# rohitgandikota/sliders

Hardware: AMD Instinct MI355X
Metric: UNet denoise steps/sec (SDXL rank-4 text slider) (higher is better)
Workload: dtype bf16; 1 GPU; sdxl text slider rank=4 alpha=1 noxattn+c3lier, 1024x1024, batch 1 (CFG pair), DDIM-50 partial denoise k~U{1..49} + 4 predictions + backward + AdamW; bench_step=one training iteration, prompt_pairs=8, parallelism=dp1

## Files before the change

sliders_amd/csrc/common.h:

```cpp
#pragma once
#include <hip/hip_runtime.h>
#include <stdint.h>

typedef __attribute__((ext_vector_type(8))) __bf16 bf16x8;
typedef __attribute__((ext_vector_type(4))) __bf16 bf16x4;
typedef __attribute__((ext_vector_type(2))) __bf16 bf16x2;
typedef __attribute__((ext_vector_type(16))) float f32x16;
typedef __attribute__((ext_vector_type(2))) float f32x2;
typedef __attribute__((ext_vector_type(4))) float f32x4;
typedef __attribute__((ext_vector_type(4))) unsigned int u32x4;
typedef __attribute__((ext_vector_type(2))) unsigned int u32x2;

typedef unsigned short bf16_t;

#define SLH_WAVE 64

static __device__ __attribute__((aligned(64))) unsigned int slh_zero_page[64];

__device__ __forceinline__ float bf2f(__bf16 x) { return (float)x; }
__device__ __forceinline__ __bf16 f2bf(float x) { return (__bf16)x; }

__device__ __forceinline__ float bfraw2f(unsigned short u) {
    return __builtin_bit_cast(float, ((unsigned int)u) << 16);
}
__device__ __forceinline__ unsigned short f2bfraw(float f) {
    return __builtin_bit_cast(unsigned short, (__bf16)f);
}
__device__ __forceinline__ float round_bf16(float f) { return (float)((__bf16)f); }

__device__ __forceinline__ float silu_f(float x) { return x / (1.0f + __expf(-x)); }
__device__ __forceinline__ float gelu_erf_f(float x) { return 0.5f * x * (1.0f + erff(x * 0.70710678118654752f)); }
__device__ __forceinline__ float gelu_erf_fast_f(float x) {
    const float z = fabsf(x) * 0.70710678118654752f;
    const float t = __builtin_amdgcn_rcpf(__builtin_fmaf(0.5f, z, 1.0f));
    float p = 0.17087277f;
    p = __builtin_fmaf(p, t, -0.82215223f); p = __builtin_fmaf(p, t, 1.48851587f); p = __builtin_fmaf(p, t, -1.13520398f);
    p = __builtin_fmaf(p, t, 0.27886807f); p = __builtin_fmaf(p, t, -0.18628806f); p = __builtin_fmaf(p, t, 0.09678418f);
    p = __builtin_fmaf(p, t, 0.37409196f); p = __builtin_fmaf(p, t, 1.00002368f); p = __builtin_fmaf(p, t, -1.26551223f);
    const float e = t * __expf(__builtin_fmaf(-z, z, p));
    const float h = 0.5f * e;
    return x * (x >= 0.f ? 1.0f - h : h);
}

__device__ __forceinline__ float wave_sum(float v) {
#pragma unroll
    for (int o = 32; o > 0; o >>= 1) v += __shfl_xor(v, o, 64);
    return v;
}
__device__ __forceinline__ float wave_max(float v) {
#pragma unroll
    for (int o = 32; o > 0; o >>= 1) v = fmaxf(v, __shfl_xor(v, o, 64));
    return v;
}

__device__ __forceinline__ void glds16(const void* gsrc, void* lds_wave_base) {
    __builtin_amdgcn_global_load_lds((const __attribute__((address_space(1))) void*)gsrc,
                                     (__attribute__((address_space(3))) void*)lds_wave_base, 16, 0, 0);
}

__device__ __forceinline__ void lds_dma_syncthreads() {
    asm volatile("s_waitcnt vmcnt(0)" ::: "memory");
    __syncthreads();
}

__device__ __forceinline__ void glds16_hidden(const void* gsrc, unsigned lds_byte_addr) {
    asm volatile("s_mov_b32 m0, %1\n\ts_nop 0\n\tglobal_load_lds_dwordx4 %0, off" ::"v"(gsrc), "s"(lds_byte_addr) : "memory");
}
__device__ __forceinline__ unsigned lds_addr_of(const void* p) {
    return (unsigned)(uintptr_t)(const __attribute__((address_space(3))) char*)p;
}
__device__ __forceinline__ int lds_off(int row, int slot) {
    return row * 128 + ((slot ^ ((row >> 1) & 7)) << 4);
}

__device__ __forceinline__ int batch_find(const int* prefix, int n, int bid) {
    int lo = 0, hi = n;
    while (hi - lo > 1) {
        const int mid = (lo + hi) >> 1;
        if (prefix[mid] <= bid) lo = mid; else hi = mid;
    }
    return lo;
// ... 142 lines not shown
#pragma unroll
            for (int u = 0; u < U; ++u) { a += (double)v[u][0]; b += (double)v[u][1]; }
        }
    }
    for (int o = lpg >> 1; o > 0; o >>= 1) {
        a += __shfl_xor(a, o, 64);
        b += __shfl_xor(b, o, 64);
    }
    S = a; Q = b;
}

__device__ __forceinline__ bool gn_cluster_reduce(const GnWorkspace ws, float* rows, unsigned* tickets, int rb, int groups, int lpg, int g,
                                                  bool owner, float S1, float Q1, int* lds_flag, double& S, double& Q) {
    const int cl = ws.cluster_of(rb);
    if (owner) store_pair_sc1(ws.pair(rows, groups, rb, g), S1, Q1);
    const int members = ws.members(cl);
    if (!last_arriver(ws.cluster_ticket(tickets, cl), (unsigned)members, lds_flag)) return false;
    gn_combine_partials(ws.pair(rows, groups, ws.first(cl), 0), members, groups, lpg, S, Q);
    return true;
}
__device__ __forceinline__ bool gn_two_level_reduce(const GnWorkspace ws, float* rows, unsigned* tickets, int rb, int groups, int lpg,
                                                    bool owner, float S1, float Q1, int* lds_flag, double& S, double& Q) {
    const int tid = threadIdx.x;
    const int g = tid / lpg;
    if (!gn_cluster_reduce(ws, rows, tickets, rb, groups, lpg, g, owner, S1, Q1, lds_flag, S, Q)) return false;
    if (ws.clusters() == 1) return g < groups && (tid & (lpg - 1)) == 0;
    if (g < groups && (tid & (lpg - 1)) == 0) store_pair_sc1(ws.pair(rows, groups, ws.cluster_row(ws.cluster_of(rb)), g), (float)S, (float)Q);
    if (!last_arriver(ws.level2_ticket(tickets), (unsigned)ws.clusters(), lds_flag)) return false;
    gn_combine_partials(ws.pair(rows, groups, ws.cluster_row(0), 0), ws.clusters(), groups, lpg, S, Q);
    return g < groups && (tid & (lpg - 1)) == 0;
}

__device__ __forceinline__ f32x2 gn_finish(double S, double Q, int hw, int cg, double pivot, float eps) {
    const double n = (double)hw * (double)cg;
    const double m = S / n;
    const double var = fmax(Q / n - m * m, 0.0);
    return f32x2{(float)(pivot + m), (float)(1.0 / sqrt(var + (double)eps))};
}

void slh_set_error(const char* fmt, ...);
#define SLH_CHECK(cond, ...)            \
    do {                                \
        if (!(cond)) {                  \
            slh_set_error(__VA_ARGS__); \
            return -1;                  \
        }                               \
    } while (0)
bool slh_name_mode();
void slh_name_record(const char* fmt, ...);
void slh_name_sink_set(char* buf, int cap);
void slh_launch_record(int grid, int block, const void* args, size_t bytes);
void slh_launch_recorded(int* grid, int* block, unsigned long long* args_hash);
inline const char* slh_tf(bool b) { return b ? "true" : "false"; }
template <auto Kern, class A, class... N>
inline void slh_launch(int grid, int block, hipStream_t s, const A& a, const char* fmt, N... n) {
    if (slh_name_mode()) { slh_name_record(fmt, n...); slh_launch_record(grid, block, &a, sizeof(A)); return; }
    hipLaunchKernelGGL(Kern, dim3(grid), dim3(block), 0, s, a);
}
#define SLH_LAUNCH_CHECK(name)                                              \
    do {                                                                    \
        if (slh_name_mode()) break;                                         \
        hipError_t e_ = hipGetLastError();                                  \
        if (e_ != hipSuccess) {                                             \
            slh_set_error("%s: launch failed: %s", name, hipGetErrorString(e_)); \
            return -2;                                                      \
        }                                                                   \
    } while (0)
```

sliders_amd/csrc/lora.hip:

```cpp
#include "addressing.h"
#include "../../include/sliders_hip.h"

namespace {

struct AddrArgs {
    const __bf16* a0; const __bf16* a1;
    int lda0, lda1, ca0, ca1;
    int mode, hs, ws, src_xform, stride, ho, wo;
};

template <int RMAX, int LPR>
__global__ __launch_bounds__(256) void skinny_kernel(AddrArgs A, const __bf16* __restrict__ w,
                                                     const __bf16* __restrict__ bias, void* out,
                                                     int M, int R, int K, int ldo, int out_kind, int kmajor) {
    const int tid = threadIdx.x;
    const int sub = tid & (LPR - 1);
    const int m = blockIdx.x * (256 / LPR) + tid / LPR;
    const bool active = m < M;
    const int mm = active ? m : M - 1;
    float acc[RMAX];
#pragma unroll
    for (int r = 0; r < RMAX; ++r) acc[r] = 0.f;
    const int cin = A.ca0 + A.ca1;

// ... 37 lines not shown
            const bf16x8 nxt = *(const bf16x8*)src_of(k + LPR * 8);
            fma_chunk(cur, k);
            cur = nxt;
        }
    } else {
        const int hw = A.ho * A.wo;
        const int b = mm / hw;
        const int rem = mm - b * hw;
        const int oy = rem / A.wo, ox = rem - oy * A.wo;
        const int sh = A.src_xform ? 1 : 0;
        const int HL = A.hs << sh, WL = A.ws << sh;
        for (int tap = 0; tap < 9; ++tap) {
            const int ky = tap / 3, kx = tap - ky * 3;
            const int iy = oy * A.stride + ky - 1, ix = ox * A.stride + kx - 1;
            bool ok = (iy >= 0) & (iy < HL) & (ix >= 0) & (ix < WL);
            if (A.src_xform == 2) ok = ok & (((iy | ix) & 1) == 0);
            if (!ok) continue;
            const long pix = ((long)b * A.hs + (iy >> sh)) * A.ws + (ix >> sh);
            auto src_of = [&](int c) {
                const int cc = c < cin ? c : 0;
                return cc < A.ca0 ? A.a0 + pix * A.lda0 + cc : A.a1 + pix * A.lda1 + (cc - A.ca0);
            };
            bf16x8 cur = *(const bf16x8*)src_of(sub * 8);
            for (int c = sub * 8; c < cin; c += LPR * 8) {
                const bf16x8 nxt = *(const bf16x8*)src_of(c + LPR * 8);
                fma_chunk(cur, tap * cin + c);
                cur = nxt;
            }
        }
    }
#pragma unroll
    for (int r = 0; r < RMAX; ++r) {
#pragma unroll
        for (int o = LPR / 2; o > 0; o >>= 1) acc[r] += __shfl_xor(acc[r], o, 64);
    }
    if (active && sub == 0) {
        if (out_kind == 0) {
            float* o = (float*)out + (long)m * ldo;
#pragma unroll
            for (int r = 0; r < RMAX; ++r)
                if (r < R) o[r] = acc[r] + (bias ? (float)bias[r] : 0.f);
        } else {
            const int hw = A.ho * A.wo;
            const int b = m / hw;
            const int rem = m - b * hw;
            __bf16* o = (__bf16*)out;
#pragma unroll
            for (int r = 0; r < RMAX; ++r)
                if (r < R) o[((long)b * R + r) * hw + rem] = (__bf16)(acc[r] + (bias ? (float)bias[r] : 0.f));
        }
    }
}

__global__ __launch_bounds__(256) void gemv_kernel(const slh_gemv_desc d) {
    const int lane = threadIdx.x & 63;
    const int n = blockIdx.x * 4 + (threadIdx.x >> 6);
    if (n >= d.N) return;
    const __bf16* x = (const __bf16*)d.x;
    const __bf16* w = (const __bf16*)d.w + (long)n * d.K;
    float acc[8];
#pragma unroll
    for (int b = 0; b < 8; ++b) acc[b] = 0.f;
    for (int k = lane * 8; k < d.K; k += 512) {
        const bf16x8 wv = *(const bf16x8*)(w + k);
        bf16x8 xv[8];
#pragma unroll
        for (int b = 0; b < 8; ++b) xv[b] = *(const bf16x8*)(x + (long)(b < d.nb ? b : d.nb - 1) * d.ldx + k);
        float wf[8];
#pragma unroll
        for (int e = 0; e < 8; ++e) wf[e] = (float)wv[e];
#pragma unroll
        for (int b = 0; b < 8; ++b) {
            if (b < d.nb) {
#pragma unroll
                for (int e = 0; e < 8; ++e) {
                    float xe = (float)xv[b][e];
                    if (d.in_act == 1) xe = round_bf16(silu_f(xe));
                    acc[b] += xe * wf[e];
                }
            }
        }
    }
#pragma unroll
    for (int b = 0; b < 8; ++b) acc[b] = wave_sum(acc[b]);
    if (lane == 0) {
        const float bias = d.bias ? (float)((const __bf16*)d.bias)[n] : 0.f;
        float up[4] = {0.f, 0.f, 0.f, 0.f};
        float ls = 0.f;
        int tcol = 0;
        if (d.lora_t) {
            ls = *d.lora_scale;
            tcol = d.lora_tcol ? d.lora_tcol[n] : 0;
            const bf16x4 u = *(const bf16x4*)((const __bf16*)d.lora_up + (long)n * 4);
#pragma unroll
            for (int r = 0; r < 4; ++r) up[r] = (float)u[r];
        }
        for (int b = 0; b < d.nb; ++b) {
            float v = acc[b] + bias;
            if (d.lora_t) {
                const float* t = d.lora_t + (long)b * d.ld_t + tcol;
                v += ls * (t[0] * up[0] + t[1] * up[1] + t[2] * up[2] + t[3] * up[3]);
            }
            if (d.addend) v = round_bf16(v) + (float)((const __bf16*)d.addend)[(long)b * d.ld_add + n];
            if (d.out_f32) ((float*)d.y)[(long)b * d.ldy + n] = v;
            else ((__bf16*)d.y)[(long)b * d.ldy + n] = (__bf16)v;
        }
    }
}

struct WgradArgs {
    AddrArgs A;
    const float* v; float* out; const float* scale;
    int M, R, ldv, ldo, rows_per_block, rmajor, vgroup_cols;
    float* ws; unsigned* ticket;
};

template <int R>
__device__ __forceinline__ void wgrad_body(const WgradArgs& p, const int bx, const int by, const int bz, const long slab_id = 0,
                                           const int slab_step = 0, const long ticket_id = 0, const int splits = 1) {
    __shared__ float red[4][32][8 * R + 1];
    __shared__ int last_flag;
    const int cx = threadIdx.x & 31, ry = threadIdx.x >> 5;
    const int C = p.A.ca0 + p.A.ca1;
    const int c = (bx * 32 + cx) * 8;
    const bool cvalid = c < C;
    const int tap = bz;
    const int m_begin = by * p.rows_per_block;
    const int m_end = min(p.M, m_begin + p.rows_per_block);
    float acc[8][R];
#pragma unroll
    for (int e = 0; e < 8; ++e)
#pragma unroll
        for (int r = 0; r < R; ++r) acc[e][r] = 0.f;
    const int voff = p.vgroup_cols > 0 ? 4 * (c / p.vgroup_cols) : 0;
    const int ky = tap / 3, kx = tap - ky * 3;
    const SrcSel zs = src_select(p.A, c);
    if (cvalid) {
        for (int m = m_begin + ry; m < m_end; m += 8) {
            long pix = m;
            if (p.A.mode != 0) {
                const RowPixel px = pixel_of_row(m, p.A.ho, p.A.wo);
                const ConvTap t = conv_tap(p.A, px.b, px.oy, px.ox, ky, kx);
                if (!t.ok) continue;
                pix = t.pix;
            }
            const bf16x8 z = *(const bf16x8*)(zs.base + pix * zs.ld + zs.cc);
            float vv[R];
#pragma unroll
            for (int r = 0; r < R; ++r) vv[r] = p.v[(long)m * p.ldv + voff + r];
#pragma unroll
            for (int e = 0; e < 8; ++e) {
                const float ze = (float)z[e];
#pragma unroll
                for (int r = 0; r < R; ++r) acc[e][r] += ze * vv[r];
// ... 108 lines not shown
    p.vgroup_cols = d.vgroup_cols;
    p.ws = d.slabs; p.ticket = (unsigned*)d.tickets;
    p.rows_per_block = wgrad_geom(d.c0 + d.c1, d.M, d.mode, d.slabs ? 1 : 0).rows_per_block;
}

template <int R>
__global__ __launch_bounds__(256) void wgrad_batch_kernel(const slh_wgrad_desc* table, const int* prefix, int n, float* ws, unsigned* ticket) {
    const int bid = blockIdx.x;
    const int pi = __builtin_amdgcn_readfirstlane(batch_find(prefix, n, bid));
    const slh_wgrad_desc d = table[pi];
    WgradArgs p;
    wgrad_args(p, d);
    p.ws = ws; p.ticket = ticket;
    const WgradGeom g = wgrad_geom(d.c0 + d.c1, d.M, d.mode, ws ? 2 : 0);
    p.rows_per_block = g.rows_per_block;
    const int local = bid - prefix[pi];
    const int bx = local % g.gx, rest = local / g.gx;
    const int by = rest % g.splits, bz = rest / g.splits;
    wgrad_body<R>(p, bx, by, bz, bid, g.gx, (long)prefix[pi] + (long)bz * g.splits * g.gx + bx, g.splits);
}

}

struct skinny_form { int rmax, lpr, grid; };
static skinny_form skinny_choose(int M, int R) {
    skinny_form f;
    f.rmax = R <= 4 ? 4 : R <= 12 ? 12 : 16;
    f.lpr = M <= 16384 ? 64 : 16;
    const int rows = 256 / f.lpr;
    f.grid = (M + rows - 1) / rows;
    return f;
}

extern "C" int slh_skinny(const slh_skinny_desc* d, slh_stream_t stream) {
    SLH_CHECK(d && d->a0 && d->w && d->out, "slh_skinny: null pointer");
    SLH_CHECK(d->M > 0 && d->R > 0 && d->R <= 16 && d->K > 0, "slh_skinny: bad shape");
    SLH_CHECK(d->ca0 % 8 == 0 && d->ca1 % 8 == 0 && d->lda0 % 8 == 0 && d->lda1 % 8 == 0 && d->K % 8 == 0,
              "slh_skinny: 16-byte alignment");
    SLH_CHECK((d->a1 != nullptr) == (d->ca1 > 0), "slh_skinny: a1/ca1 mismatch");
    const int cin = d->ca0 + d->ca1;
    if (d->mode == 0) SLH_CHECK(cin == d->K, "slh_skinny: dense K mismatch");
    else {
        SLH_CHECK(d->mode == 1 && d->K == 9 * cin, "slh_skinny: conv K mismatch");
        SLH_CHECK(d->M == d->batch * d->ho * d->wo, "slh_skinny: conv M mismatch");
        SLH_CHECK(d->stride == 1 || d->stride == 2, "slh_skinny: stride");
    }
    if (d->out_kind == 1) SLH_CHECK(d->mode == 1, "slh_skinny: NCHW output needs conv geometry");
    if (d->w_kmajor) SLH_CHECK(d->R == 4 && d->mode == 0 && !d->bias, "slh_skinny: w_kmajor needs dense R=4");
    AddrArgs A;
    fill_addr(A, d->a0, d->a1, d->lda0, d->lda1, d->ca0, d->ca1, d->mode, d->hs, d->ws, d->src_xform, d->stride,
              d->ho, d->wo);
    hipStream_t s = (hipStream_t)stream;
    const skinny_form f = skinny_choose(d->M, d->R);
#define SLH_SKINNY_LAUNCH(RM, LPR)                                                                                 \
    do {                                                                                                           \
        if (slh_name_mode()) slh_name_record("skinny<%d,%d>", RM, LPR);                                            \
        else                                                                                                       \
            hipLaunchKernelGGL((skinny_kernel<RM, LPR>), dim3(f.grid), dim3(256), 0, s, A, (const __bf16*)d->w,    \
                               (const __bf16*)d->bias, d->out, d->M, d->R, d->K, d->ldo, d->out_kind, d->w_kmajor); \
    } while (0)
#define SLH_SKINNY_ROWS(RM)                                                                                        \
    do {                                                                                                           \
        if (f.lpr == 64) SLH_SKINNY_LAUNCH(RM, 64);                                                                \
        else SLH_SKINNY_LAUNCH(RM, 16);                                                                            \
    } while (0)
    if (f.rmax == 4) SLH_SKINNY_ROWS(4);
    else if (f.rmax == 12) SLH_SKINNY_ROWS(12);
    else SLH_SKINNY_ROWS(16);
#undef SLH_SKINNY_ROWS
#undef SLH_SKINNY_LAUNCH
    SLH_LAUNCH_CHECK("slh_skinny");
    return 0;
}

extern "C" int slh_skinny_kernel_name(const slh_skinny_desc* d, char* buf, int cap) {
    SLH_CHECK(buf && cap >= 32, "slh_skinny_kernel_name: buffer");
    slh_name_sink_set(buf, cap);
    const int rc = slh_skinny(d, nullptr);
    slh_name_sink_set(nullptr, 0);
    if (rc == 0 && !buf[0]) { slh_set_error("slh_skinny_kernel_name: internal: no launch site recorded a name"); return -3; }
    return rc;
}

extern "C" int slh_gemv(const slh_gemv_desc* d, slh_stream_t stream) {
    SLH_CHECK(d && d->x && d->w && d->y, "slh_gemv: null pointer");
    SLH_CHECK(d->nb >= 1 && d->nb <= 8 && d->N > 0 && d->K > 0 && d->K % 8 == 0 && d->ldx % 8 == 0,
              "slh_gemv: bad shape nb=%d N=%d K=%d", d->nb, d->N, d->K);
    if (d->lora_t) SLH_CHECK(d->lora_up && d->lora_scale, "slh_gemv: lora pointers");
    hipLaunchKernelGGL(gemv_kernel, dim3((d->N + 3) / 4), dim3(256), 0, (hipStream_t)stream, *d);
    SLH_LAUNCH_CHECK("slh_gemv");
    return 0;
}

static int wgrad_check(const slh_wgrad_desc* d, bool ptrs = true) {
    SLH_CHECK(d, "slh_lora_wgrad: null descriptor");
    if (ptrs) SLH_CHECK(d->z0 && d->v && d->out && d->scale, "slh_lora_wgrad: null pointer");
    SLH_CHECK(d->R == 4 || d->R == 12, "slh_lora_wgrad: R must be 4 or 12");
    SLH_CHECK(d->c0 % 8 == 0 && d->c1 % 8 == 0 && d->ldz0 % 8 == 0 && d->ldz1 % 8 == 0, "slh_lora_wgrad: alignment");
    if (ptrs) SLH_CHECK((d->z1 != nullptr) == (d->c1 > 0), "slh_lora_wgrad: z1/c1 mismatch");
    SLH_CHECK(d->M > 0 && d->c0 + d->c1 > 0, "slh_lora_wgrad: empty problem");
    if (d->mode == 1) SLH_CHECK(d->M == d->batch * d->ho * d->wo, "slh_lora_wgrad: conv M mismatch");
    if (d->vgroup_cols > 0)
        SLH_CHECK(d->vgroup_cols % 8 == 0 && (d->c0 + d->c1) % d->vgroup_cols == 0 && d->R == 4,
                  "slh_lora_wgrad: vgroup_cols %d needs a multiple of 8 that divides C = %d, and R = 4 (R = %d)", d->vgroup_cols,
                  d->c0 + d->c1, d->R);
    SLH_CHECK(d->vgroup_cols >= 0, "slh_lora_wgrad: negative vgroup_cols");
    return 0;
}

extern "C" int slh_lora_wgrad(const slh_wgrad_desc* d, slh_stream_t stream) {
    if (wgrad_check(d)) return -1;
    WgradArgs p;
    wgrad_args(p, *d);
    SLH_CHECK((d->slabs != nullptr) == (d->tickets != nullptr), "slh_lora_wgrad: slabs and tickets come together");
    const WgradGeom g = wgrad_geom(d->c0 + d->c1, d->M, d->mode, d->slabs ? 1 : 0);
    dim3 grid(g.gx, g.splits, g.taps);
    hipStream_t s = (hipStream_t)stream;
    if (d->R == 4) hipLaunchKernelGGL(wgrad_kernel<4>, grid, dim3(256), 0, s, p);
    else hipLaunchKernelGGL(wgrad_kernel<12>, grid, dim3(256), 0, s, p);
    SLH_LAUNCH_CHECK("slh_lora_wgrad");
    return 0;
}

extern "C" int slh_lora_wgrad_blocks(const slh_wgrad_desc* d) {
    if (wgrad_check(d, false)) return -1;
    const WgradGeom g = wgrad_geom(d->c0 + d->c1, d->M, d->mode, d->slabs ? 2 : 0);
    return g.gx * g.splits * g.taps;
}

extern "C" int slh_lora_wgrad_single_blocks(const slh_wgrad_desc* d) {
    if (wgrad_check(d, false)) return -1;
    const WgradGeom g = wgrad_geom(d->c0 + d->c1, d->M, d->mode, 1);
    return g.gx * g.splits * g.taps;
}

extern "C" int slh_lora_wgrad_geometry(const slh_wgrad_desc* d, int kind, int32_t* out4) {
    if (wgrad_check(d, false)) return -1;
    SLH_CHECK(kind >= 0 && kind <= 2 && out4, "slh_lora_wgrad_geometry: kind must be 0, 1 or 2");
    const WgradGeom g = wgrad_geom(d->c0 + d->c1, d->M, d->mode, kind);
    out4[0] = g.gx; out4[1] = g.splits; out4[2] = g.taps; out4[3] = g.rows_per_block;
    return 0;
}
// ... 147 lines not shown
```

sliders_amd/csrc/ops.hip:

```cpp
#include "common.h"
#include "../../include/sliders_hip.h"

namespace {

__global__ void tembed_kernel(const slh_tembed_desc d) {
    const int idx = blockIdx.x * blockDim.x + threadIdx.x;
    const int per = d.n_vals * d.dim;
    if (idx >= d.nb * per) return;
    const int b = idx / per;
    const int rem = idx - b * per;
    const int j = rem / d.dim;
    const int i = rem - j * d.dim;
    const int half = d.dim / 2;
    const int fi = i < half ? i : i - half;
    const float exponent = (-9.210340371976184f * (float)fi) / (float)half;
    const float arg = d.vals[b * d.n_vals + j] * expf(exponent);
    const float v = i < half ? cosf(arg) : sinf(arg);
    ((__bf16*)d.out)[(long)b * d.ldo + d.col0 + rem] = (__bf16)v;
}

constexpr int CONVIN_ITERS = 8;
__global__ void conv_in_kernel(const slh_convin_desc d, int nchunk, int ppb) {
    extern __shared__ __attribute__((aligned(16))) char cin_smem[];
    __bf16* sw = (__bf16*)cin_smem;
// ... 8 lines not shown
    const long npix = (long)d.batch * hw;
    float bias[8];
#pragma unroll
    for (int e = 0; e < 8; ++e) bias[e] = d.bias ? (float)((const __bf16*)d.bias)[chunk * 8 + e] : 0.f;
    for (int it = 0; it < CONVIN_ITERS; ++it) {
        const long pix = ((long)blockIdx.x * CONVIN_ITERS + it) * ppb + pl;
        if (pix >= npix) break;
        const int b = (int)(pix / hw);
        const int rem = (int)(pix - (long)b * hw);
        const int oy = rem / d.wd, ox = rem - oy * d.wd;
        const __bf16* x = (const __bf16*)d.x + (long)b * d.cin * hw;
        float acc[8];
#pragma unroll
        for (int e = 0; e < 8; ++e) acc[e] = bias[e];
        if (d.cin <= 4) {
            __bf16 xin[9][4];
            bool tin[9];
#pragma unroll
            for (int tap = 0; tap < 9; ++tap) {
                const int iy = oy + tap / 3 - 1, ix = ox + tap % 3 - 1;
                tin[tap] = iy >= 0 && iy < d.h && ix >= 0 && ix < d.wd;
                const int cy = iy < 0 ? 0 : (iy >= d.h ? d.h - 1 : iy), cx = ix < 0 ? 0 : (ix >= d.wd ? d.wd - 1 : ix);
#pragma unroll
                for (int ci = 0; ci < 4; ++ci) xin[tap][ci] = x[(long)(ci < d.cin ? ci : 0) * hw + cy * d.wd + cx];
            }
#pragma unroll
            for (int tap = 0; tap < 9; ++tap) {
                if (!tin[tap]) continue;
#pragma unroll
                for (int ci = 0; ci < 4; ++ci) {
                    if (ci >= d.cin) break;
                    const float xv = (float)xin[tap][ci];
                    const bf16x8 wv = *(const bf16x8*)(sw + (tap * d.cin + ci) * d.cout + chunk * 8);
#pragma unroll
                    for (int e = 0; e < 8; ++e) acc[e] += xv * (float)wv[e];
                }
            }
        } else {
            for (int tap = 0; tap < 9; ++tap) {
                const int iy = oy + tap / 3 - 1, ix = ox + tap % 3 - 1;
                if (iy < 0 || iy >= d.h || ix < 0 || ix >= d.wd) continue;
                for (int ci = 0; ci < d.cin; ++ci) {
                    const float xv = (float)x[(long)ci * hw + iy * d.wd + ix];
                    const bf16x8 wv = *(const bf16x8*)(sw + (tap * d.cin + ci) * d.cout + chunk * 8);
#pragma unroll
                    for (int e = 0; e < 8; ++e) acc[e] += xv * (float)wv[e];
                }
            }
        }
        bf16x8 o;
#pragma unroll
        for (int e = 0; e < 8; ++e) o[e] = (__bf16)acc[e];
        *(bf16x8*)((__bf16*)d.y + pix * d.ldy + chunk * 8) = o;
    }
}

__global__ __launch_bounds__(256) void ew_kernel(const slh_ew_desc d) {
    const int nchunk = d.C / 8;
    const long gid = (long)blockIdx.x * blockDim.x + threadIdx.x;
    if (gid >= (long)d.M * nchunk) return;
    const int chunk = (int)(gid % nchunk);
    const long m = gid / nchunk;
    const int c = chunk * 8;
    const __bf16* A = (const __bf16*)d.a;
    const __bf16* B = (const __bf16*)d.b;
    __bf16* O = (__bf16*)d.out;
    if (d.op == SLH_EW_COPY) {
        *(bf16x8*)(O + m * d.ldo + c) = *(const bf16x8*)(A + m * d.lda + c);
    } else if (d.op == SLH_EW_ADD) {
        const bf16x8 x = *(const bf16x8*)(A + m * d.lda + c);
        const bf16x8 y = *(const bf16x8*)(B + m * d.ldb + c);
        bf16x8 o;
#pragma unroll
        for (int e = 0; e < 8; ++e) o[e] = (__bf16)((float)x[e] + (float)y[e]);
        *(bf16x8*)(O + m * d.ldo + c) = o;
    } else if (d.op == SLH_EW_GEGLU_FWD || d.op == SLH_EW_GEGLU_BWD) {
        const int jb = c >> 5, j = c & 31;
        const __bf16* pa = A + m * d.lda + jb * 64 + j;
        const bf16x8 hv = *(const bf16x8*)pa;
        const bf16x8 gv = *(const bf16x8*)(pa + 32);
        if (d.op == SLH_EW_GEGLU_FWD) {
            bf16x8 o;
#pragma unroll
            for (int e = 0; e < 8; ++e) o[e] = (__bf16)((float)hv[e] * round_bf16(gelu_erf_fast_f((float)gv[e])));
            *(bf16x8*)(O + m * d.ldo + c) = o;
        } else {
            const bf16x8 dy = *(const bf16x8*)(B + m * d.ldb + c);
            bf16x8 dh, dg;
#pragma unroll
            for (int e = 0; e < 8; ++e) {
                const float g = (float)gv[e], hh = (float)hv[e], dd = (float)dy[e];
                const float cdf = 0.5f * (1.f + erff(g * 0.70710678118654752f));
                const float pdf = 0.3989422804014327f * __expf(-0.5f * g * g);
                dh[e] = (__bf16)(dd * round_bf16(g * cdf));
                dg[e] = (__bf16)(round_bf16(dd * hh) * (cdf + g * pdf));
            }
            __bf16* po = O + m * d.ldo + jb * 64 + j;
            *(bf16x8*)po = dh;
            *(bf16x8*)(po + 32) = dg;
        }
    } else if (d.op == SLH_EW_UPSAMPLE_BWD) {
        const int w = d.iarg, hw = d.iarg2;
        const long b = m / hw;
        const int rem = (int)(m - b * hw);
        const int y = rem / w, x = rem - y * w;
        const long base = (b * 4 * hw + (long)(2 * y) * (2 * w) + 2 * x);
// ... 131 lines not shown
__global__ __launch_bounds__(256) void adamw_f32_kernel(const slh_adamw_desc d, float decay, float bc2_sqrt,
                                                        float neg_step_size, float w1, float beta2, float w2, float eps) {
    const long i = (long)blockIdx.x * blockDim.x + threadIdx.x;
    if (i >= d.n) return;
    float* P = (float*)d.param; float* M1 = (float*)d.exp_avg; float* M2 = (float*)d.exp_avg_sq;
    const float g = d.grad_scale == 1.0f ? d.grad[i] : d.grad[i] * d.grad_scale;
    float p = P[i] * decay;
    float m = M1[i];
    m = __builtin_fmaf(w1, g - m, m);
    float v = M2[i] * beta2;
    v = __builtin_fmaf(w2, g * g, v);
    float den = __builtin_sqrtf(v);
    den = den / bc2_sqrt;
    den = den + eps;
    p = __builtin_fmaf(neg_step_size, m / den, p);
    P[i] = p; M1[i] = m; M2[i] = v;
    ((__bf16*)d.param_lo)[i] = (__bf16)p;
}

__global__ __launch_bounds__(256) void lion_kernel(const slh_lion_desc d, float decay, float b1, float w1, float b2,
                                                   float w2, float neg_lr) {
    const long i = (long)blockIdx.x * blockDim.x + threadIdx.x;
    if (i >= d.n) return;
    __bf16* P = (__bf16*)d.param; __bf16* M = (__bf16*)d.exp_avg;
    const float g = round_bf16(d.grad[i] * d.grad_scale);
    float p = round_bf16((float)P[i] * decay);
    const float m0 = (float)M[i];
    float u = round_bf16(m0 * b1);
    u = round_bf16(u + w1 * g);
    const float sg = u > 0.f ? 1.f : (u < 0.f ? -1.f : 0.f);
    p = round_bf16(p + neg_lr * sg);
    float m = round_bf16(m0 * b2);
    m = round_bf16(m + w2 * g);
    P[i] = (__bf16)p; M[i] = (__bf16)m;
}

}

extern "C" int slh_timestep_embed(const slh_tembed_desc* d, slh_stream_t stream) {
    SLH_CHECK(d && d->vals && d->out && d->dim % 2 == 0 && d->nb > 0 && d->n_vals > 0, "slh_timestep_embed: bad desc");
    const int total = d->nb * d->n_vals * d->dim;
    hipLaunchKernelGGL(tembed_kernel, dim3((total + 255) / 256), dim3(256), 0, (hipStream_t)stream, *d);
    SLH_LAUNCH_CHECK("slh_timestep_embed");
    return 0;
}

extern "C" int slh_conv_in(const slh_convin_desc* d, slh_stream_t stream) {
    SLH_CHECK(d && d->x && d->w && d->y, "slh_conv_in: null pointer");
    SLH_CHECK(d->cout % 8 == 0 && d->ldy % 8 == 0 && d->cin > 0 && d->cin <= 16, "slh_conv_in: bad shape");
    const int nchunk = d->cout / 8;
    SLH_CHECK(nchunk <= 256 && 9 * d->cin * d->cout * 2 <= 64 * 1024, "slh_conv_in: weights must fit 64 KB of LDS");
    const int ppb = 256 / nchunk;
    const long npix = (long)d->batch * d->h * d->wd;
    const long per_block = (long)ppb * CONVIN_ITERS;
    hipLaunchKernelGGL(conv_in_kernel, dim3((unsigned)((npix + per_block - 1) / per_block)), dim3(nchunk * ppb),
                       9 * d->cin * d->cout * 2, (hipStream_t)stream, *d, nchunk, ppb);
    SLH_LAUNCH_CHECK("slh_conv_in");
    return 0;
}

extern "C" int slh_elementwise(const slh_ew_desc* d, slh_stream_t stream) {
    SLH_CHECK(d && d->a && d->out, "slh_elementwise: null pointer");
    SLH_CHECK(d->C % 8 == 0 && d->lda % 8 == 0 && d->ldo % 4 == 0, "slh_elementwise: alignment");
    hipStream_t s = (hipStream_t)stream;
    if (d->op == SLH_EW_COLSUM) {
        SLH_CHECK(d->iarg2 > 0 && d->M % d->iarg2 == 0, "slh_elementwise: colsum rows per sample");
        dim3 grid((d->C / 8 + 31) / 32, (d->iarg2 + 511) / 512, d->M / d->iarg2);
        hipLaunchKernelGGL(colsum_kernel, grid, dim3(256), 0, s, *d);
    } else {
        if (d->op == SLH_EW_ADD || d->op == SLH_EW_GEGLU_BWD) SLH_CHECK(d->b && d->ldb % 8 == 0, "slh_elementwise: operand b");
        if (d->op == SLH_EW_GEGLU_FWD || d->op == SLH_EW_GEGLU_BWD) SLH_CHECK(d->C % 32 == 0, "slh_elementwise: geglu C");
        if (d->op == SLH_EW_UPSAMPLE_BWD) SLH_CHECK(d->iarg > 0 && d->iarg2 > 0, "slh_elementwise: upsample dims");
        const long total = (long)d->M * (d->C / 8);
        hipLaunchKernelGGL(ew_kernel, dim3((unsigned)((total + 255) / 256)), dim3(256), 0, s, *d);
    }
    SLH_LAUNCH_CHECK("slh_elementwise");
    return 0;
}

namespace {
__global__ __launch_bounds__(256) void gather16_kernel(const unsigned short* src, const int* idx, unsigned short* out, long n) {
    const long i = (long)blockIdx.x * blockDim.x + threadIdx.x;
    if (i >= n) return;
    const int j = idx[i];
    out[i] = j < 0 ? (unsigned short)0 : src[j];
}
}

extern "C" int slh_gather16(const slh_gather16_desc* d, slh_stream_t stream) {
    SLH_CHECK(d && d->src && d->idx && d->out && d->n > 0, "slh_gather16: null pointer / empty");
    hipLaunchKernelGGL(gather16_kernel, dim3((unsigned)((d->n + 255) / 256)), dim3(256), 0, (hipStream_t)stream,
                       (const unsigned short*)d->src, d->idx, (unsigned short*)d->out, (long)d->n);
    SLH_LAUNCH_CHECK("slh_gather16");
    return 0;
}

extern "C" int slh_cfg_ddim(const slh_cfg_ddim_desc* d, slh_stream_t stream) {
    SLH_CHECK(d && d->eps && d->out && (d->x || !d->do_step), "slh_cfg_ddim: null pointer");
    const long n = (long)d->nb * d->chw;
    hipLaunchKernelGGL(cfg_ddim_kernel, dim3((unsigned)((n + 255) / 256)), dim3(256), 0, (hipStream_t)stream, *d);
    SLH_LAUNCH_CHECK("slh_cfg_ddim");
    return 0;
}

extern "C" int slh_guidance_loss(const slh_loss_desc* d, slh_stream_t stream) {
    SLH_CHECK(d && d->target && d->positive && d->neutral && d->uncond && d->loss, "slh_guidance_loss: null pointer");
// ... 35 lines not shown
```

Baseline: 45.96 steps/s.

## Add specialized kernels for LoRA 3x3 skinny conv, wide GEMV, and conv_in

Adds three new kernel paths behind an SLH_SMALL_OPS switch that is on by default. The first is a skinny 3x3 conv kernel for rank-4 LoRA down-projections, with fp32 weights held in LDS and register prefetch of the next tap. The second is a wide GEMV that gives each wave four output rows, stages x in LDS, and prefetches weights. The third is a persistent conv_in kernel with fp32 LDS weights, double-buffered input tiles, and an interior fast path. Each targets the latency and bandwidth limits of small ops. The trade-off is higher LDS use, and arithmetic ordering that mimics the old rounding through contract-off multiplies, which the unusual mixed FMA in the skinny kernel suggests was tuned for bitwise matching.

```diff
diff --git a/sliders_amd/csrc/common.h b/sliders_amd/csrc/common.h
--- a/sliders_amd/csrc/common.h
+++ b/sliders_amd/csrc/common.h
@@ -1,6 +1,7 @@
 #pragma once
 #include <hip/hip_runtime.h>
 #include <stdint.h>
+#include <stdlib.h>
 
 typedef __attribute__((ext_vector_type(8))) __bf16 bf16x8;
 typedef __attribute__((ext_vector_type(4))) __bf16 bf16x4;
@@ -27,6 +28,16 @@
     return __builtin_bit_cast(unsigned short, (__bf16)f);
 }
 __device__ __forceinline__ float round_bf16(float f) { return (float)((__bf16)f); }
+
+__device__ __forceinline__ float mul_rn(float a, float b) {
+#pragma clang fp contract(off)
+    return a * b;
+}
+__device__ __forceinline__ float mul_add_rn(float a, float b, float c) {
+#pragma clang fp contract(off)
+    const float p = a * b;
+    return p + c;
+}
 
 __device__ __forceinline__ float silu_f(float x) { return x / (1.0f + __expf(-x)); }
 __device__ __forceinline__ float gelu_erf_f(float x) { return 0.5f * x * (1.0f + erff(x * 0.70710678118654752f)); }
@@ -275,6 +286,10 @@
 void slh_launch_record(int grid, int block, const void* args, size_t bytes);
 void slh_launch_recorded(int* grid, int* block, unsigned long long* args_hash);
 inline const char* slh_tf(bool b) { return b ? "true" : "false"; }
+inline int slh_small_ops() {
+    static const int v = getenv("SLH_SMALL_OPS") ? atoi(getenv("SLH_SMALL_OPS")) : 1;
+    return v;
+}
 template <auto Kern, class A, class... N>
 inline void slh_launch(int grid, int block, hipStream_t s, const A& a, const char* fmt, N... n) {
     if (slh_name_mode()) { slh_name_record(fmt, n...); slh_launch_record(grid, block, &a, sizeof(A)); return; }
diff --git a/sliders_amd/csrc/lora.hip b/sliders_amd/csrc/lora.hip
--- a/sliders_amd/csrc/lora.hip
+++ b/sliders_amd/csrc/lora.hip
@@ -113,6 +113,149 @@
     }
 }
 
+constexpr int SKC_J = 3;
+constexpr int SKC_ROWS = 32;
+constexpr int SKC_MAX_GRID = 512;
+__global__ __launch_bounds__(256) void skinny_conv16_kernel(AddrArgs A, const __bf16* __restrict__ w,
+                                                            const __bf16* __restrict__ bias, void* out,
+                                                            int M, int R, int K, int ldo, int out_kind) {
+    extern __shared__ __attribute__((aligned(16))) char skc_smem[];
+    f32x4* sw = (f32x4*)skc_smem;
+    const int tid = threadIdx.x;
+    const int K8 = K / 8;
+    {
+        bf16x8 v[4][2];
+#pragma unroll
+        for (int r = 0; r < 4; ++r)
+#pragma unroll
+            for (int u = 0; u < 2; ++u) {
+                const int q = tid + u * 256;
+                v[r][u] = *(const bf16x8*)(w + (long)(r < R ? r : 0) * K + (q < K8 ? q : 0) * 8);
+            }
+#pragma unroll
+        for (int r = 0; r < 4; ++r)
+#pragma unroll
+            for (int u = 0; u < 2; ++u) {
+                const int q = tid + u * 256;
+                if (r < R && q < K8) {
+                    sw[(r * 2 + 0) * K8 + q] = f32x4{(float)v[r][u][0], (float)v[r][u][1], (float)v[r][u][2], (float)v[r][u][3]};
+                    sw[(r * 2 + 1) * K8 + q] = f32x4{(float)v[r][u][4], (float)v[r][u][5], (float)v[r][u][6], (float)v[r][u][7]};
+                }
+            }
+    }
+    __syncthreads();
+    const int sub = tid & 15, grp = tid >> 4;
+    const int cin = A.ca0 + A.ca1;
+    const int hw = A.ho * A.wo;
+    const int sh = A.src_xform ? 1 : 0;
+    const int HL = A.hs << sh, WL = A.ws << sh;
+    for (long base = (long)blockIdx.x * SKC_ROWS; base < M; base += (long)gridDim.x * SKC_ROWS) {
+        int m[2], b[2], oy[2], ox[2];
+#pragma unroll
+        for (int p = 0; p < 2; ++p) {
+            m[p] = (int)base + p * 16 + grp;
+            const int mm = m[p] < M ? m[p] : M - 1;
+            b[p] = mm / hw;
+            const int rem = mm - b[p] * hw;
+            oy[p] = rem / A.wo;
+            ox[p] = rem - oy[p] * A.wo;
+        }
+        float acc[2][4];
+#pragma unroll
+        for (int p = 0; p < 2; ++p)
+#pragma unroll
+            for (int r = 0; r < 4; ++r) acc[p][r] = 0.f;
+        bf16x8 cur[2][SKC_J], nxt[2][SKC_J];
+        bool okc[2], okn[2];
+        auto fetch = [&](int tap, bf16x8 (&dst)[2][SKC_J], bool (&ok)[2]) {
+            const int ky = tap / 3, kx = tap - ky * 3;
+#pragma unroll
+            for (int p = 0; p < 2; ++p) {
+                const int iy = oy[p] * A.stride + ky - 1, ix = ox[p] * A.stride + kx - 1;
+                ok[p] = (iy >= 0) & (iy < HL) & (ix >= 0) & (ix < WL);
+                if (A.src_xform == 2) ok[p] = ok[p] & (((iy | ix) & 1) == 0);
+                const int cy = iy < 0 ? 0 : (iy >= HL ? HL - 1 : iy), cx = ix < 0 ? 0 : (ix >= WL ? WL - 1 : ix);
+                const long pix = ((long)b[p] * A.hs + (cy >> sh)) * A.ws + (cx >> sh);
+#pragma unroll
+                for (int j = 0; j < SKC_J; ++j) {
+                    const int c = sub * 8 + j * 128;
+                    const int cc = c < cin ? c : 0;
+                    dst[p][j] = *(const bf16x8*)(cc < A.ca0 ? A.a0 + pix * A.lda0 + cc : A.a1 + pix * A.lda1 + (cc - A.ca0));
+                }
+            }
+        };
+        fetch(0, cur, okc);
+#pragma unroll 1
+        for (int tap = 0; tap < 9; ++tap) {
+            if (tap < 8) fetch(tap + 1, nxt, okn);
+#pragma unroll
+            for (int j = 0; j < SKC_J; ++j) {
+                const int c = sub * 8 + j * 128;
+                if (c < cin && (okc[0] | okc[1])) {
+                    const int q = (tap * cin + c) >> 3;
+                    float wf[4][8];
+#pragma unroll
+                    for (int r = 0; r < 4; ++r) {
+                        const int rr = r < R ? r : 0;
+                        const f32x4 w0 = sw[(rr * 2 + 0) * K8 + q], w1 = sw[(rr * 2 + 1) * K8 + q];
+#pragma unroll
+                        for (int e = 0; e < 4; ++e) { wf[r][e] = w0[e]; wf[r][4 + e] = w1[e]; }
+                    }
+#pragma unroll
+                    for (int p = 0; p < 2; ++p) {
+                        if (okc[p]) {
+                            float xf[8];
+#pragma unroll
+                            for (int e = 0; e < 8; ++e) xf[e] = (float)cur[p][j][e];
+#pragma unroll
+                            for (int r = 0; r < 4; ++r) {
+                                if (r < R) {
+#pragma unroll
+                                    for (int e = 0; e < 8; ++e)
+                                        acc[p][r] = r == 3 && (e & 1) == 0 ? __builtin_fmaf(xf[e], wf[r][e], acc[p][r])
+                                                                           : mul_add_rn(xf[e], wf[r][e], acc[p][r]);
+                                }
+                            }
+                        }
+                    }
+                }
+            }
+            if (tap < 8) {
+#pragma unroll
+                for (int p = 0; p < 2; ++p) {
+                    okc[p] = okn[p];
+#pragma unroll
+                    for (int j = 0; j < SKC_J; ++j) cur[p][j] = nxt[p][j];
+                }
+            }
+        }
+#pragma unroll
+        for (int p = 0; p < 2; ++p) {
+            float a[4];
+#pragma unroll
+            for (int r = 0; r < 4; ++r) {
+                a[r] = acc[p][r];
+#pragma unroll
+                for (int o = 8; o > 0; o >>= 1) a[r] += __shfl_xor(a[r], o, 64);
+            }
+            if (m[p] < M && sub == 0) {
+                if (out_kind == 0) {
+                    float* o = (float*)out + (long)m[p] * ldo;
+#pragma unroll
+                    for (int r = 0; r < 4; ++r)
+                        if (r < R) o[r] = a[r] + (bias ? (float)bias[r] : 0.f);
+                } else {
+                    const int rem = m[p] - b[p] * hw;
+                    __bf16* o = (__bf16*)out;
+#pragma unroll
+                    for (int r = 0; r < 4; ++r)
+                        if (r < R) o[((long)b[p] * R + r) * hw + rem] = (__bf16)(a[r] + (bias ? (float)bias[r] : 0.f));
+                }
+            }
+        }
+    }
+}
+
 __global__ __launch_bounds__(256) void gemv_kernel(const slh_gemv_desc d) {
     const int lane = threadIdx.x & 63;
     const int n = blockIdx.x * 4 + (threadIdx.x >> 6);
@@ -161,6 +304,118 @@
             if (d.lora_t) {
                 const float* t = d.lora_t + (long)b * d.ld_t + tcol;
                 v += ls * (t[0] * up[0] + t[1] * up[1] + t[2] * up[2] + t[3] * up[3]);
+            }
+            if (d.addend) v = round_bf16(v) + (float)((const __bf16*)d.addend)[(long)b * d.ld_add + n];
+            if (d.out_f32) ((float*)d.y)[(long)b * d.ldy + n] = v;
+            else ((__bf16*)d.y)[(long)b * d.ldy + n] = (__bf16)v;
+        }
+    }
+}
+
+constexpr int GEMV_F = 4;
+constexpr int GEMV_S = 3;
+__global__ __launch_bounds__(256) void gemv_wide_kernel(const slh_gemv_desc d) {
+    extern __shared__ __attribute__((aligned(16))) char gemv_smem[];
+    bf16x8* sx = (bf16x8*)gemv_smem;
+    const int lane = threadIdx.x & 63;
+    const int n0 = (blockIdx.x * 4 + (threadIdx.x >> 6)) * GEMV_F;
+    const int K8 = d.K / 8;
+    const __bf16* w[GEMV_F];
+#pragma unroll
+    for (int f = 0; f < GEMV_F; ++f) w[f] = (const __bf16*)d.w + (long)(n0 + f < d.N ? n0 + f : d.N - 1) * d.K;
+    bf16x8 wv[GEMV_F][GEMV_S];
+    auto request = [&](int k0) {
+#pragma unroll
+        for (int s = 0; s < GEMV_S; ++s) {
+            const int k = k0 + s * 512 + lane * 8;
+#pragma unroll
+            for (int f = 0; f < GEMV_F; ++f) wv[f][s] = *(const bf16x8*)(w[f] + (k < d.K ? k : 0));
+        }
+    };
+    const int nx = d.nb * K8;
+    auto piece = [&](int i) {
+        const int b = i / K8, q = i - b * K8;
+        return *(const bf16x8*)((const __bf16*)d.x + (long)b * d.ldx + q * 8);
+    };
+    auto staged = [&](bf16x8 v) {
+        if (d.in_act == 1) {
+#pragma unroll
+            for (int e = 0; e < 8; ++e) v[e] = (__bf16)silu_f((float)v[e]);
+        }
+        return v;
+    };
+    const bf16x8 x0 = piece(threadIdx.x < nx ? threadIdx.x : 0);
+    request(0);
+    if (threadIdx.x < nx) sx[threadIdx.x] = staged(x0);
+    for (int i = threadIdx.x + 256; i < nx; i += 256) sx[i] = staged(piece(i));
+    __syncthreads();
+    float acc[GEMV_F][8];
+#pragma unroll
+    for (int f = 0; f < GEMV_F; ++f)
+#pragma unroll
+        for (int b = 0; b < 8; ++b) acc[f][b] = 0.f;
+    for (int k0 = 0;;) {
+#pragma unroll
+        for (int s = 0; s < GEMV_S; ++s) {
+            const int k = k0 + s * 512 + lane * 8;
+            if (k < d.K) {
+                float wf[GEMV_F][8];
+#pragma unroll
+                for (int f = 0; f < GEMV_F; ++f)
+#pragma unroll
+                    for (int e = 0; e < 8; ++e) wf[f][e] = (float)wv[f][s][e];
+#pragma unroll
+                for (int b = 0; b < 8; ++b) {
+                    if (b < d.nb) {
+                        const bf16x8 xv = sx[b * K8 + (k >> 3)];
+#pragma unroll
+                        for (int e = 0; e < 8; ++e) {
+                            const float xe = (float)xv[e];
+#pragma unroll
+                            for (int f = 0; f < GEMV_F; ++f) acc[f][b] = __builtin_fmaf(xe, wf[f][e], acc[f][b]);
+                        }
+                    }
+                }
+            }
+        }
+        k0 += GEMV_S * 512;
+        if (k0 >= d.K) break;
+        request(k0);
+    }
+#pragma unroll
+    for (int b = 0; b < 8; ++b) {
+        if (b < d.nb) {
+#pragma unroll
+            for (int f = 0; f < GEMV_F; ++f) acc[f][b] = wave_sum(acc[f][b]);
+        }
+    }
+    if (lane < GEMV_F && n0 + lane < d.N) {
+        const int n = n0 + lane;
+        float a[8];
+#pragma unroll
+        for (int b = 0; b < 8; ++b) {
+            a[b] = acc[0][b];
+#pragma unroll
+            for (int f = 1; f < GEMV_F; ++f) a[b] = lane == f ? acc[f][b] : a[b];
+        }
+        const float bias = d.bias ? (float)((const __bf16*)d.bias)[n] : 0.f;
+        float up[4] = {0.f, 0.f, 0.f, 0.f};
+        float ls = 0.f;
+        int tcol = 0;
+        if (d.lora_t) {
+            ls = *d.lora_scale;
+            tcol = d.lora_tcol ? d.lora_tcol[n] : 0;
+            const bf16x4 u = *(const bf16x4*)((const __bf16*)d.lora_up + (long)n * 4);
+#pragma unroll
+            for (int r = 0; r < 4; ++r) up[r] = (float)u[r];
+        }
+#pragma unroll
+        for (int b = 0; b < 8; ++b) {
+            if (b >= d.nb) break;
+            float v = a[b] + bias;
+            if (d.lora_t) {
+                const float* t = d.lora_t + (long)b * d.ld_t + tcol;
+                v = __builtin_fmaf(ls, mul_add_rn(t[3], up[3], mul_add_rn(t[2], up[2], mul_add_rn(t[1], up[1], mul_rn(t[0], up[0])))), v);
             }
             if (d.addend) v = round_bf16(v) + (float)((const __bf16*)d.addend)[(long)b * d.ld_add + n];
             if (d.out_f32) ((float*)d.y)[(long)b * d.ldy + n] = v;
@@ -375,7 +630,17 @@
               d->ho, d->wo);
     hipStream_t s = (hipStream_t)stream;
     const skinny_form f = skinny_choose(d->M, d->R);
-#define SLH_SKINNY_LAUNCH(RM, LPR)                                                                                 \
+    if (slh_small_ops() && d->mode == 1 && f.rmax == 4 && f.lpr == 16 && cin <= 128 * SKC_J && d->R * d->K * 4 <= 64 * 1024) {
+        if (slh_name_mode()) slh_name_record("skinny<%d,%d>", 4, 16);
+        else {
+            const int trips = (d->M + SKC_ROWS - 1) / SKC_ROWS;
+            hipLaunchKernelGGL(skinny_conv16_kernel, dim3(trips < SKC_MAX_GRID ? trips : SKC_MAX_GRID), dim3(256), d->R * d->K * 4, s,
+                               A, (const __bf16*)d->w, (const __bf16*)d->bias, d->out, d->M, d->R, d->K, d->ldo, d->out_kind);
+        }
+        SLH_LAUNCH_CHECK("slh_skinny");
+        return 0;
+    }
+#define SLH_SKINNY_LAUNCH(RM, LPR)                                                                                \
     do {                                                                                                           \
         if (slh_name_mode()) slh_name_record("skinny<%d,%d>", RM, LPR);                                            \
         else                                                                                                       \
@@ -410,7 +675,11 @@
     SLH_CHECK(d->nb >= 1 && d->nb <= 8 && d->N > 0 && d->K > 0 && d->K % 8 == 0 && d->ldx % 8 == 0,
               "slh_gemv: bad shape nb=%d N=%d K=%d", d->nb, d->N, d->K);
     if (d->lora_t) SLH_CHECK(d->lora_up && d->lora_scale, "slh_gemv: lora pointers");
-    hipLaunchKernelGGL(gemv_kernel, dim3((d->N + 3) / 4), dim3(256), 0, (hipStream_t)stream, *d);
+    const long x_bytes = (long)d->nb * d->K * 2;
+    if (x_bytes <= 64 * 1024 && (slh_small_ops() == 2 || (slh_small_ops() == 1 && d->N >= 2 * 1024 * GEMV_F)))
+        hipLaunchKernelGGL(gemv_wide_kernel, dim3((d->N + 4 * GEMV_F - 1) / (4 * GEMV_F)), dim3(256), (unsigned)x_bytes, (hipStream_t)stream, *d);
+    else
+        hipLaunchKernelGGL(gemv_kernel, dim3((d->N + 3) / 4), dim3(256), 0, (hipStream_t)stream, *d);
     SLH_LAUNCH_CHECK("slh_gemv");
     return 0;
 }
diff --git a/sliders_amd/csrc/ops.hip b/sliders_amd/csrc/ops.hip
--- a/sliders_amd/csrc/ops.hip
+++ b/sliders_amd/csrc/ops.hip
@@ -84,6 +84,142 @@
 #pragma unroll
         for (int e = 0; e < 8; ++e) o[e] = (__bf16)acc[e];
         *(bf16x8*)((__bf16*)d.y + pix * d.ldy + chunk * 8) = o;
+    }
+}
+
+constexpr int CONVIN_GRID = 512;
+constexpr int CONVIN_PPB = 32;
+constexpr int CONVIN_AHEAD = 4;
+template <int CI, int P>
+__global__ __launch_bounds__(256) void conv_in_kernel2(const slh_convin_desc d, int nchunk, int ppb, int wvec, int wt, int trips) {
+    constexpr int E = 9 * CI;
+    typedef __attribute__((ext_vector_type(CI))) float xrow;
+    extern __shared__ __attribute__((aligned(16))) char cin_smem[];
+    float* sw = (float*)cin_smem;
+    const int K = 9 * d.cin;
+    const int tile = ppb * P * E;
+    float* xs = sw + K * d.cout;
+    auto w_at = [&](int k, int co) { return ((((co >> 2) & 1) * K + k) * nchunk + (co >> 3)) * 4 + (co & 3); };
+    const int hw = d.h * d.wd;
+    const int npix = d.batch * hw;
+    const int nt = blockDim.x;
+    auto fetch = [&](int trip, int e) {
+        const int slot = e / E, r = e - slot * E;
+        const int tap = r / CI, ci = r - tap * CI;
+        const unsigned pix = (unsigned)trip * (ppb * P) + slot;
+        const unsigned pc = pix < (unsigned)npix ? pix : npix - 1;
+        const int b = pc / (unsigned)hw;
+        const int rem = pc - b * hw;
+        const int oy = (unsigned)rem / (unsigned)d.wd, ox = rem - oy * d.wd;
+        const int iy = oy + tap / 3 - 1, ix = ox + tap % 3 - 1;
+        const int cy = iy < 0 ? 0 : (iy >= d.h ? d.h - 1 : iy), cx = ix < 0 ? 0 : (ix >= d.wd ? d.wd - 1 : ix);
+        return ((const __bf16*)d.x)[((long)b * d.cin + (ci < d.cin ? ci : 0)) * hw + cy * d.wd + cx];
+    };
+    __bf16 ahead[CONVIN_AHEAD];
+    auto request = [&](int trip) {
+#pragma unroll
+        for (int i = 0; i < CONVIN_AHEAD; ++i) {
+            const int e = threadIdx.x + i * nt;
+            ahead[i] = fetch(trip, e < tile ? e : tile - 1);
+        }
+    };
+    auto deliver = [&](int trip, float* dst) {
+#pragma unroll
+        for (int i = 0; i < CONVIN_AHEAD; ++i) {
+            const int e = threadIdx.x + i * nt;
+            if (e < tile) dst[e] = (float)ahead[i];
+        }
+        for (int e = threadIdx.x + CONVIN_AHEAD * nt; e < tile; e += nt) dst[e] = (float)fetch(trip, e);
+    };
+    if (blockIdx.x < trips) request(blockIdx.x);
+    if (wvec) {
+        for (int co = threadIdx.x; co < d.cout; co += nt) {
+            const bf16x4* row = (const bf16x4*)((const __bf16*)d.w + (long)co * K);
+            for (int q = 0; q < K / 4; ++q) {
+                const bf16x4 v = row[q];
+#pragma unroll
+                for (int e = 0; e < 4; ++e) sw[w_at(q * 4 + e, co)] = (float)v[e];
+            }
+        }
+    } else {
+        for (int co = threadIdx.x; co < d.cout; co += nt)
+            for (int k = 0; k < K; ++k) sw[w_at(k, co)] = (float)((const __bf16*)d.w)[(long)co * K + k];
+    }
+    const int chunk = threadIdx.x % nchunk, pl = threadIdx.x / nchunk;
+    float bias[8];
+#pragma unroll
+    for (int e = 0; e < 8; ++e) bias[e] = d.bias ? (float)((const __bf16*)d.bias)[chunk * 8 + e] : 0.f;
+    const __amdgpu_buffer_rsrc_t yr = wt_rsrc(d.y);
+    int buf = 0;
+    for (int trip = blockIdx.x; trip < trips; trip += gridDim.x, buf ^= 1) {
+        float* xt = xs + buf * tile;
+        deliver(trip, xt);
+        __syncthreads();
+        if (trip + gridDim.x < trips) request(trip + gridDim.x);
+        unsigned pix[P];
+        xrow xin[P][9];
+        bool tin[P][9];
+        bool inside = true;
+#pragma unroll
+        for (int p = 0; p < P; ++p) {
+            const int slot = p * ppb + pl;
+            pix[p] = (unsigned)trip * (ppb * P) + slot;
+            const unsigned pc = pix[p] < (unsigned)npix ? pix[p] : npix - 1;
+            const int b = pc / (unsigned)hw;
+            const int rem = pc - b * hw;
+            const int oy = (unsigned)rem / (unsigned)d.wd, ox = rem - oy * d.wd;
+#pragma unroll
+            for (int tap = 0; tap < 9; ++tap) {
+                const int iy = oy + tap / 3 - 1, ix = ox + tap % 3 - 1;
+                tin[p][tap] = iy >= 0 && iy < d.h && ix >= 0 && ix < d.wd;
+                inside = inside & tin[p][tap];
+                xin[p][tap] = *(const xrow*)(xt + slot * E + tap * CI);
+            }
+        }
+        float acc[P][8];
+#pragma unroll
+        for (int p = 0; p < P; ++p)
+#pragma unroll
+            for (int e = 0; e < 8; ++e) acc[p][e] = bias[e];
+        auto accumulate = [&](auto tested) {
+#pragma unroll
+            for (int tap = 0; tap < 9; ++tap) {
+                if constexpr (decltype(tested)::value) {
+                    bool any = false;
+#pragma unroll
+                    for (int p = 0; p < P; ++p) any = any | tin[p][tap];
+                    if (!any) continue;
+                }
+#pragma unroll
+                for (int ci = 0; ci < CI; ++ci) {
+                    if (ci < d.cin) {
+                        const int k = tap * d.cin + ci;
+                        const f32x4 w0 = *(const f32x4*)(sw + (k * nchunk + chunk) * 4), w1 = *(const f32x4*)(sw + ((K + k) * nchunk + chunk) * 4);
+                        const float wf[8] = {w0[0], w0[1], w0[2], w0[3], w1[0], w1[1], w1[2], w1[3]};
+#pragma unroll
+                        for (int p = 0; p < P; ++p) {
+                            if (!decltype(tested)::value || tin[p][tap]) {
+                                const float xv = xin[p][tap][ci];
+#pragma unroll
+                                for (int e = 0; e < 8; ++e) acc[p][e] = __builtin_fmaf(xv, wf[e], acc[p][e]);
+                            }
+                        }
+                    }
+                }
+            }
+        };
+        if (__all(inside)) accumulate(std::false_type{});
+        else accumulate(std::true_type{});
+#pragma unroll
+        for (int p = 0; p < P; ++p) {
+            if (pix[p] < (unsigned)npix) {
+                bf16x8 o;
+#pragma unroll
+                for (int e = 0; e < 8; ++e) o[e] = (__bf16)acc[p][e];
+                if (wt) wt_store16(yr, ((long)pix[p] * d.ldy + chunk * 8) * 2, o);
+                else *(bf16x8*)((__bf16*)d.y + (long)pix[p] * d.ldy + chunk * 8) = o;
+            }
+        }
     }
 }
 
@@ -321,6 +457,23 @@
     SLH_CHECK(nchunk <= 256 && 9 * d->cin * d->cout * 2 <= 64 * 1024, "slh_conv_in: weights must fit 64 KB of LDS");
     const int ppb = 256 / nchunk;
     const long npix = (long)d->batch * d->h * d->wd;
+    const int P = d->cin <= 4 ? 2 : 1, CI = d->cin <= 4 ? 4 : 16;
+    const int ppb2 = ppb < CONVIN_PPB ? ppb : CONVIN_PPB;
+    const int lds2 = (9 * d->cin * d->cout + 2 * ppb2 * P * 9 * CI) * 4;
+    if (slh_small_ops() && lds2 <= 64 * 1024 && npix + 2 * 256 < 0x7FFFFFFFL) {
+        const int K = 9 * d->cin;
+        const int wvec = ((uintptr_t)d->w & 7) == 0 && K % 4 == 0;
+        const int wt = ((uintptr_t)d->y & 15) == 0 && wt_span_ok(npix, d->ldy, d->cout);
+        const int trips = (int)((npix + (long)ppb2 * P - 1) / ((long)ppb2 * P));
+        const int per = (trips + CONVIN_GRID - 1) / CONVIN_GRID;
+        const dim3 grid((unsigned)((trips + per - 1) / per)), block(nchunk * ppb2);
+        if (d->cin <= 4)
+            hipLaunchKernelGGL((conv_in_kernel2<4, 2>), grid, block, lds2, (hipStream_t)stream, *d, nchunk, ppb2, wvec, wt, trips);
+        else
+            hipLaunchKernelGGL((conv_in_kernel2<16, 1>), grid, block, lds2, (hipStream_t)stream, *d, nchunk, ppb2, wvec, wt, trips);
+        SLH_LAUNCH_CHECK("slh_conv_in");
+        return 0;
+    }
     const long per_block = (long)ppb * CONVIN_ITERS;
     hipLaunchKernelGGL(conv_in_kernel, dim3((unsigned)((npix + per_block - 1) / per_block)), dim3(nchunk * ppb),
                        9 * d->cin * d->cout * 2, (hipStream_t)stream, *d, nchunk, ppb);
```

Measured after the change: 45.95 steps/s. About the same (-0.0%).
